# davide-coccomini/MINTIME-Multi-Identity-size-iNvariant-TIMEsformer-for-Video-Deepfake-Detection

Measured on AMD Instinct MI355X. Metric: clips/sec (8-frame, 2-identity, 224^2 crops) fwd+bwd, higher is better.
Workload: dtype f32; 1 GPU; config 3: EfficientNet-B0 + SizeInvariantTimeSformer(dim 512, depth 9, heads 8), B=32/GPU, 8 frames, 2 identities (identity-masked), 224x224 crops, random-init seeded weights (restored before every step), train-mode BN + drop-connect 0.2, step = fwd + BCE loss + bwd + SGD(lr .01, wd 1e-4); global_batch=32, frames=8, parallelism=dp1

## Files before the change

### mintime-multi-identity-size-invariant-timesformer-for-video-deepfake-detection_amd/csrc/tsf_bwd.hip

```cpp
#include "../../include/mintime_hip.h"
#include "common.hpp"
#include <stdlib.h>
#include <float.h>

using namespace mt;

#include "planes.hpp"
#include "det.hpp"
namespace {

constexpr int DH = 64;

template <int NI>
__global__ __launch_bounds__(256) void layernorm_bwd_kernel(const float* __restrict__ dy, const float* __restrict__ x,
                                                            const float* __restrict__ stats, const float* __restrict__ gamma,
                                                            float* __restrict__ dx, float* __restrict__ dgamma,
                                                            float* __restrict__ dbeta, int rows, int D, int accumulate,
                                                            float* __restrict__ dxsum, int skip_period, const float* dx_in, const DetLog det) {
  const int lane = threadIdx.x & 63;
  const int wave_global = blockIdx.x * 4 + (threadIdx.x >> 6);
  const int nwaves = gridDim.x * 4;
  const int nq = D >> 2;
  float4 dg[NI], db[NI], g[NI], ds[NI];
#pragma unroll
  for (int i = 0; i < NI; ++i) {
    dg[i] = make_float4(0.f, 0.f, 0.f, 0.f); db[i] = dg[i]; ds[i] = dg[i];
    const int q = lane + i * 64;
    g[i] = q < nq ? reinterpret_cast<const float4*>(gamma)[q] : make_float4(0.f, 0.f, 0.f, 0.f);
  }
  for (int row0 = wave_global; row0 < rows; row0 += 2 * nwaves) {
    const int row1 = row0 + nwaves;
    const bool has1 = row1 < rows;
    const int r1 = has1 ? row1 : row0;
    const float mean0 = stats[2 * (int64_t)row0], rstd0 = stats[2 * (int64_t)row0 + 1];
    const float mean1 = stats[2 * (int64_t)r1], rstd1 = stats[2 * (int64_t)r1 + 1];
    const float4* xr0 = reinterpret_cast<const float4*>(x + (int64_t)row0 * D);
    const float4* dyr0 = reinterpret_cast<const float4*>(dy + (int64_t)row0 * D);
    const float4* xr1 = reinterpret_cast<const float4*>(x + (int64_t)r1 * D);
    const float4* dyr1 = reinterpret_cast<const float4*>(dy + (int64_t)r1 * D);
    float4 xh0[NI], gy0[NI], xh1[NI], gy1[NI];
    float a1 = 0.f, a2 = 0.f, b1 = 0.f, b2 = 0.f;
    const float w1 = has1 ? 1.f : 0.f;
#pragma unroll
    for (int i = 0; i < NI; ++i) {
      const int q = lane + i * 64;
      if (q < nq) {
        const float4 xv0 = xr0[q], d0 = dyr0[q], xv1 = xr1[q], d1 = dyr1[q];
        xh0[i] = make_float4((xv0.x - mean0) * rstd0, (xv0.y - mean0) * rstd0, (xv0.z - mean0) * rstd0, (xv0.w - mean0) * rstd0);
        xh1[i] = make_float4((xv1.x - mean1) * rstd1, (xv1.y - mean1) * rstd1, (xv1.z - mean1) * rstd1, (xv1.w - mean1) * rstd1);
        gy0[i] = make_float4(d0.x * g[i].x, d0.y * g[i].y, d0.z * g[i].z, d0.w * g[i].w);
        gy1[i] = make_float4(d1.x * g[i].x, d1.y * g[i].y, d1.z * g[i].z, d1.w * g[i].w);
        a1 += gy0[i].x + gy0[i].y + gy0[i].z + gy0[i].w;
        a2 += gy0[i].x * xh0[i].x + gy0[i].y * xh0[i].y + gy0[i].z * xh0[i].z + gy0[i].w * xh0[i].w;
        b1 += gy1[i].x + gy1[i].y + gy1[i].z + gy1[i].w;
        b2 += gy1[i].x * xh1[i].x + gy1[i].y * xh1[i].y + gy1[i].z * xh1[i].z + gy1[i].w * xh1[i].w;
        dg[i].x += d0.x * xh0[i].x + w1 * d1.x * xh1[i].x; dg[i].y += d0.y * xh0[i].y + w1 * d1.y * xh1[i].y;
        dg[i].z += d0.z * xh0[i].z + w1 * d1.z * xh1[i].z; dg[i].w += d0.w * xh0[i].w + w1 * d1.w * xh1[i].w;
        db[i].x += d0.x + w1 * d1.x; db[i].y += d0.y + w1 * d1.y; db[i].z += d0.z + w1 * d1.z; db[i].w += d0.w + w1 * d1.w;
      }
    }
    a1 = wave_sum(a1) / (float)D; a2 = wave_sum(a2) / (float)D;
    b1 = wave_sum(b1) / (float)D; b2 = wave_sum(b2) / (float)D;
    float4* dxr0 = reinterpret_cast<float4*>(dx + (int64_t)row0 * D);
    float4* dxr1 = reinterpret_cast<float4*>(dx + (int64_t)r1 * D);
    const float4* pin0 = reinterpret_cast<const float4*>(dx_in + (int64_t)row0 * D);
    const float4* pin1 = reinterpret_cast<const float4*>(dx_in + (int64_t)r1 * D);
    const float c0 = (skip_period > 0 && row0 % skip_period == 0) ? 0.f : 1.f;
    const float c1 = (!has1 || (skip_period > 0 && row1 % skip_period == 0)) ? 0.f : 1.f;
#pragma unroll
    for (int i = 0; i < NI; ++i) {
      const int q = lane + i * 64;
      if (q < nq) {
        float4 o;
        o.x = rstd0 * (gy0[i].x - a1 - xh0[i].x * a2); o.y = rstd0 * (gy0[i].y - a1 - xh0[i].y * a2);
        o.z = rstd0 * (gy0[i].z - a1 - xh0[i].z * a2); o.w = rstd0 * (gy0[i].w - a1 - xh0[i].w * a2);
        if (accumulate) { const float4 p = pin0[q]; o.x += p.x; o.y += p.y; o.z += p.z; o.w += p.w; }
        dxr0[q] = o;
        ds[i].x += c0 * o.x; ds[i].y += c0 * o.y; ds[i].z += c0 * o.z; ds[i].w += c0 * o.w;
        if (has1) {
          float4 t;
          t.x = rstd1 * (gy1[i].x - b1 - xh1[i].x * b2); t.y = rstd1 * (gy1[i].y - b1 - xh1[i].y * b2);
          t.z = rstd1 * (gy1[i].z - b1 - xh1[i].z * b2); t.w = rstd1 * (gy1[i].w - b1 - xh1[i].w * b2);
          if (accumulate) { const float4 p = pin1[q]; t.x += p.x; t.y += p.y; t.z += p.z; t.w += p.w; }
          dxr1[q] = t;
          ds[i].x += c1 * t.x; ds[i].y += c1 * t.y; ds[i].z += c1 * t.z; ds[i].w += c1 * t.w;
        }
      }
    }
  }
  __shared__ float red[4][1024];
  const int wv = threadIdx.x >> 6;
#pragma unroll 1
  for (int which = 0; which < 3; ++which) {
    if (which == 2 && !dxsum) break;
#pragma unroll
    for (int i = 0; i < NI; ++i) {
      const int q = lane + i * 64;
      if (q < nq) *reinterpret_cast<float4*>(&red[wv][4 * q]) = which == 0 ? dg[i] : (which == 1 ? db[i] : ds[i]);
    }
    __syncthreads();
    float* dst = which == 0 ? dgamma : (which == 1 ? dbeta : dxsum);
    for (int c = threadIdx.x; c < D; c += 256) {
      const float v = red[0][c] + red[1][c] + red[2][c] + red[3][c];
      if (det.vals) det_put(det, which, blockIdx.x, c, v);
      else atomicAdd(dst + c, v);
    }
    __syncthreads();
  }
}

template <int NI, bool KEEP = false>
__device__ __forceinline__ void layernorm_bwd_rows_body(const float* __restrict__ dy, const float* __restrict__ x,
                                                        const float* __restrict__ stats, const float* __restrict__ gamma,
                                                        float* __restrict__ dx, const float* __restrict__ dx_in, int rows, int D,
                                                        const PlaneRef dxp) {
  const int lane = threadIdx.x & 63;
  const int nwaves = gridDim.x * 4;
  const int nq = D >> 2;
  const float inv_d = 1.0f / (float)D;
  if (dxp.p && blockIdx.x == 0)
    for (int row = rows + (threadIdx.x >> 6); row < dxp.rows_pad; row += 4)
      for (int q = lane; q < nq; q += 64) planes_store4(dxp, row, q * 4, 0.f, 0.f, 0.f, 0.f);
  for (int row = blockIdx.x * 4 + (threadIdx.x >> 6); row < rows; row += nwaves) {
    const float mean = stats[2 * (int64_t)row], rstd = stats[2 * (int64_t)row + 1];
    const float4* xr = reinterpret_cast<const float4*>(x + (int64_t)row * D);
    const float4* dyr = reinterpret_cast<const float4*>(dy + (int64_t)row * D);
    const float4* pin = reinterpret_cast<const float4*>(dx_in + (int64_t)row * D);
    float4* dxr = reinterpret_cast<float4*>(dx + (int64_t)row * D);
    if constexpr (KEEP) {
      float4 xv[NI], d[NI], g[NI], pv[NI];
      float a1 = 0.f, a2 = 0.f;
#pragma unroll
      for (int i = 0; i < NI; ++i) {
        const int q = min(lane + i * 64, nq - 1);
        xv[i] = xr[q]; d[i] = dyr[q]; g[i] = reinterpret_cast<const float4*>(gamma)[q]; pv[i] = pin[q];
      }
#pragma unroll
      for (int i = 0; i < NI; ++i) {
        const float w = lane + i * 64 < nq ? 1.f : 0.f;
        const float gx = d[i].x * g[i].x, gy_ = d[i].y * g[i].y, gz = d[i].z * g[i].z, gw = d[i].w * g[i].w;
        a1 += w * (gx + gy_ + gz + gw);
        a2 += w * rstd * (gx * (xv[i].x - mean) + gy_ * (xv[i].y - mean) + gz * (xv[i].z - mean) + gw * (xv[i].w - mean));
      }
      a1 = wave_sum(a1) * inv_d; a2 = wave_sum(a2) * inv_d;
#pragma unroll
      for (int i = 0; i < NI; ++i) {
        const int q = lane + i * 64;
        if (q < nq) {
          float4 o;
          o.x = rstd * (d[i].x * g[i].x - a1 - (xv[i].x - mean) * rstd * a2) + pv[i].x; o.y = rstd * (d[i].y * g[i].y - a1 - (xv[i].y - mean) * rstd * a2) + pv[i].y;
          o.z = rstd * (d[i].z * g[i].z - a1 - (xv[i].z - mean) * rstd * a2) + pv[i].z; o.w = rstd * (d[i].w * g[i].w - a1 - (xv[i].w - mean) * rstd * a2) + pv[i].w;
          dxr[q] = o;
          if (dxp.p) planes_store4(dxp, row, q * 4, o.x, o.y, o.z, o.w);
        }
      }
      continue;
    }
    float a1 = 0.f, a2 = 0.f;
#pragma unroll 1
    for (int i = 0; i < NI; ++i) {
      const int q = min(lane + i * 64, nq - 1);
      const float w = lane + i * 64 < nq ? 1.f : 0.f;
      const float4 xv = xr[q], d = dyr[q], g = reinterpret_cast<const float4*>(gamma)[q];
      const float gx = d.x * g.x, gy_ = d.y * g.y, gz = d.z * g.z, gw = d.w * g.w;
      a1 += w * (gx + gy_ + gz + gw);
      a2 += w * rstd * (gx * (xv.x - mean) + gy_ * (xv.y - mean) + gz * (xv.z - mean) + gw * (xv.w - mean));
    }
    a1 = wave_sum(a1) * inv_d; a2 = wave_sum(a2) * inv_d;
#pragma unroll 1
    for (int i = 0; i < NI; ++i) {
      const int q = lane + i * 64;
      if (q < nq) {
        const float4 xv = xr[q], d = dyr[q], g = reinterpret_cast<const float4*>(gamma)[q], p = pin[q];
        float4 o;
        o.x = rstd * (d.x * g.x - a1 - (xv.x - mean) * rstd * a2) + p.x; o.y = rstd * (d.y * g.y - a1 - (xv.y - mean) * rstd * a2) + p.y;
        o.z = rstd * (d.z * g.z - a1 - (xv.z - mean) * rstd * a2) + p.z; o.w = rstd * (d.w * g.w - a1 - (xv.w - mean) * rstd * a2) + p.w;
        dxr[q] = o;
        if (dxp.p) planes_store4(dxp, row, q * 4, o.x, o.y, o.z, o.w);
      }
    }
  }
}

__global__ __launch_bounds__(256) void layernorm_bwd_rows_kernel2k(
    const float* dy, const float* x, const float* stats, const float* gamma, float* dx, const float* dx_in, int rows, int D, PlaneRef dxp) {
  layernorm_bwd_rows_body<2, true>(dy, x, stats, gamma, dx, dx_in, rows, D, dxp);
}
__global__ __launch_bounds__(256) void layernorm_bwd_rows_kernel4(const float* dy, const float* x, const float* stats, const float* gamma,
                                                                   float* dx, const float* dx_in, int rows, int D, PlaneRef dxp) {
  layernorm_bwd_rows_body<4>(dy, x, stats, gamma, dx, dx_in, rows, D, dxp);
}

__global__ __launch_bounds__(256) void layernorm_bwd_rows_sums_kernel(
    const float* __restrict__ dy, const float* __restrict__ x, const float* __restrict__ stats, const float* __restrict__ gamma,
    float* __restrict__ dx, const float* __restrict__ dx_in, int rows, int D, PlaneRef dxp, float* __restrict__ partials, int skip_period) {
  constexpr int NI = 2;
  const int lane = threadIdx.x & 63, wv = threadIdx.x >> 6;
  const int nwaves = gridDim.x * 4;
  const int nq = D >> 2;
  const float inv_d = 1.0f / (float)D;
  if (dxp.p && blockIdx.x == 0)
    for (int row = rows + wv; row < dxp.rows_pad; row += 4)
      for (int q = lane; q < nq; q += 64) planes_store4(dxp, row, q * 4, 0.f, 0.f, 0.f, 0.f);
  float4 dg[NI], db[NI], ds[NI];
#pragma unroll
  for (int i = 0; i < NI; ++i) { dg[i] = make_float4(0.f, 0.f, 0.f, 0.f); db[i] = dg[i]; ds[i] = dg[i]; }
  for (int row = blockIdx.x * 4 + wv; row < rows; row += nwaves) {
    const float mean = stats[2 * (int64_t)row], rstd = stats[2 * (int64_t)row + 1];
    const float keep = (skip_period > 0 && row % skip_period == 0) ? 0.f : 1.f;
    const float4* xr = reinterpret_cast<const float4*>(x + (int64_t)row * D);
    const float4* dyr = reinterpret_cast<const float4*>(dy + (int64_t)row * D);
    const float4* pin = reinterpret_cast<const float4*>(dx_in + (int64_t)row * D);
    float4* dxr = reinterpret_cast<float4*>(dx + (int64_t)row * D);
    float4 xv[NI], d[NI], g[NI], pv[NI];
    float a1 = 0.f, a2 = 0.f;
#pragma unroll
    for (int i = 0; i < NI; ++i) {
      const int q = min(lane + i * 64, nq - 1);
      xv[i] = xr[q]; d[i] = dyr[q]; g[i] = reinterpret_cast<const float4*>(gamma)[q]; pv[i] = pin[q];
    }
#pragma unroll
    for (int i = 0; i < NI; ++i) {
      const float w = lane + i * 64 < nq ? 1.f : 0.f;
      xv[i].x = (xv[i].x - mean) * rstd; xv[i].y = (xv[i].y - mean) * rstd; xv[i].z = (xv[i].z - mean) * rstd; xv[i].w = (xv[i].w - mean) * rstd;
      const float gx = d[i].x * g[i].x, gy_ = d[i].y * g[i].y, gz = d[i].z * g[i].z, gw = d[i].w * g[i].w;
      a1 += w * (gx + gy_ + gz + gw);
      a2 += w * (gx * xv[i].x + gy_ * xv[i].y + gz * xv[i].z + gw * xv[i].w);
    }
    a1 = wave_sum(a1) * inv_d; a2 = wave_sum(a2) * inv_d;
#pragma unroll
    for (int i = 0; i < NI; ++i) {
      const int q = lane + i * 64;
      if (q < nq) {
        float4 o;
        o.x = rstd * (d[i].x * g[i].x - a1 - xv[i].x * a2) + pv[i].x; o.y = rstd * (d[i].y * g[i].y - a1 - xv[i].y * a2) + pv[i].y;
        o.z = rstd * (d[i].z * g[i].z - a1 - xv[i].z * a2) + pv[i].z; o.w = rstd * (d[i].w * g[i].w - a1 - xv[i].w * a2) + pv[i].w;
        dxr[q] = o;
        if (dxp.p) planes_store4(dxp, row, q * 4, o.x, o.y, o.z, o.w);
        dg[i].x += d[i].x * xv[i].x; dg[i].y += d[i].y * xv[i].y; dg[i].z += d[i].z * xv[i].z; dg[i].w += d[i].w * xv[i].w;
        db[i].x += d[i].x; db[i].y += d[i].y; db[i].z += d[i].z; db[i].w += d[i].w;
        ds[i].x += keep * o.x; ds[i].y += keep * o.y; ds[i].z += keep * o.z; ds[i].w += keep * o.w;
      }
    }
  }
  __shared__ float red[4][512];
  auto meet = [&](const float4 (&v)[NI], int which) {
#pragma unroll
    for (int i = 0; i < NI; ++i) {
      const int q = lane + i * 64;
      if (q < nq) *reinterpret_cast<float4*>(&red[wv][4 * q]) = v[i];
    }
    __syncthreads();
    float* dst = partials + ((int64_t)blockIdx.x * 3 + which) * D;
    for (int c = threadIdx.x; c < D; c += 256) dst[c] = red[0][c] + red[1][c] + red[2][c] + red[3][c];
    __syncthreads();
  };
  meet(dg, 0);
  meet(db, 1);
  meet(ds, 2);
}

__global__ __launch_bounds__(1024) void layernorm_cols_reduce_kernel(const float* __restrict__ partials, int blocks, int D,
                                                                     float* __restrict__ dgamma, float* __restrict__ dbeta,
                                                                     float* __restrict__ dxsum) {
  const int which = blockIdx.y;
  float* dst = which == 0 ? dgamma : (which == 1 ? dbeta : dxsum);
  if (!dst) return;
  __shared__ float red[16][64];
  const int cl = threadIdx.x & 63, ph = threadIdx.x >> 6;
  const int c = blockIdx.x * 64 + cl;
  float s0 = 0.f, s1 = 0.f, s2 = 0.f, s3 = 0.f;
  if (c < D) {
    const float* src = partials + (int64_t)which * D + c;
    const int64_t stride = (int64_t)3 * D;
    int b = ph;
    for (; b + 48 < blocks; b += 64) {
      s0 += src[(int64_t)b * stride]; s1 += src[(int64_t)(b + 16) * stride];
      s2 += src[(int64_t)(b + 32) * stride]; s3 += src[(int64_t)(b + 48) * stride];
    }
    for (; b < blocks; b += 16) s0 += src[(int64_t)b * stride];
  }
  red[ph][cl] = (s0 + s1) + (s2 + s3);
  __syncthreads();
  if (ph == 0 && c < D) {
    float t = 0.f;
#pragma unroll
    for (int q = 0; q < 16; ++q) t += red[q][cl];
    dst[c] += t;
  }
}

template <int NI>
__global__ __launch_bounds__(256) void layernorm_bwd_cols_kernel(const float* __restrict__ dy, const float* __restrict__ x,
                                                                 const float* __restrict__ stats, const float* __restrict__ dxn,
                                                                 float* __restrict__ dgamma, float* __restrict__ dbeta,
                                                                 float* __restrict__ dxsum, int skip_period, int rows, int D, const DetLog det) {
  const int lane = threadIdx.x & 63;
  const int nwaves = gridDim.x * 4;
  const int nq = D >> 2;
  float4 dg[NI], db[NI], ds[NI];
#pragma unroll
  for (int i = 0; i < NI; ++i) { dg[i] = make_float4(0.f, 0.f, 0.f, 0.f); db[i] = dg[i]; ds[i] = dg[i]; }
  for (int row = blockIdx.x * 4 + (threadIdx.x >> 6); row < rows; row += nwaves) {
    const float mean = stats[2 * (int64_t)row], rstd = stats[2 * (int64_t)row + 1];
    const float c = (skip_period > 0 && row % skip_period == 0) ? 0.f : 1.f;
#pragma unroll
    for (int i = 0; i < NI; ++i) {
      const int q = lane + i * 64;
      if (q < nq) {
        const float4 xv = reinterpret_cast<const float4*>(x + (int64_t)row * D)[q];
        const float4 d = reinterpret_cast<const float4*>(dy + (int64_t)row * D)[q];
        dg[i].x += d.x * ((xv.x - mean) * rstd); dg[i].y += d.y * ((xv.y - mean) * rstd);
        dg[i].z += d.z * ((xv.z - mean) * rstd); dg[i].w += d.w * ((xv.w - mean) * rstd);
        db[i].x += d.x; db[i].y += d.y; db[i].z += d.z; db[i].w += d.w;
        if (dxsum) {
          const float4 o = reinterpret_cast<const float4*>(dxn + (int64_t)row * D)[q];
          ds[i].x += c * o.x; ds[i].y += c * o.y; ds[i].z += c * o.z; ds[i].w += c * o.w;
        }
      }
    }
  }
  __shared__ float red[4][1024];
  const int wv = threadIdx.x >> 6;
#pragma unroll 1
  for (int which = 0; which < 3; ++which) {
    if (which == 2 && !dxsum) break;
#pragma unroll
    for (int i = 0; i < NI; ++i) {
      const int q = lane + i * 64;
      if (q < nq) *reinterpret_cast<float4*>(&red[wv][4 * q]) = which == 0 ? dg[i] : (which == 1 ? db[i] : ds[i]);
    }
    __syncthreads();
    float* dst = which == 0 ? dgamma : (which == 1 ? dbeta : dxsum);
    for (int cidx = threadIdx.x; cidx < D; cidx += 256) {
      const float v = red[0][cidx] + red[1][cidx] + red[2][cidx] + red[3][cidx];
      if (det.vals) det_put(det, which, blockIdx.x, cidx, v);
      else atomicAdd(dst + cidx, v);
    }
    __syncthreads();
  }
}

__global__ __launch_bounds__(256) void colsum_kernel(const float* __restrict__ A, int64_t lda, int gin, int gout, int off,
                                                     int M, int N, float* __restrict__ out, int rows_per_block, const DetLog det) {
  __shared__ float red[4][64];
  const int cl = threadIdx.x & 63, rl = threadIdx.x >> 6;
  const int n = blockIdx.x * 64 + cl;
  const int m0 = blockIdx.y * rows_per_block;
  const int m1 = min(M, m0 + rows_per_block);
  float s = 0.f;
  if (n < N) {
    for (int m = m0 + rl; m < m1; m += 4) {
      int64_t r = m;
      if (gin) { const int g = m / gin; r = (int64_t)g * gout + off + (m - g * gin); }
      s += A[r * lda + n];
    }
  }
  red[rl][cl] = s;
  __syncthreads();
  if (rl == 0 && n < N) {
    const float v = red[0][cl] + red[1][cl] + red[2][cl] + red[3][cl];
    if (det.vals) {
      det_put(det, blockIdx.x, blockIdx.y, cl, v);
      if (blockIdx.y == 0 && cl == 0) det_base(det, blockIdx.x, (int64_t)blockIdx.x * 64);
    } else atomicAdd(out + n, v);
  }
}

__global__ void head_bwd_kernel(const float* __restrict__ dlogits, const float* __restrict__ x, const float* __restrict__ gamma,
                                const float* __restrict__ beta, const float* __restrict__ w, float* __restrict__ dx,
                                float* __restrict__ dgamma, float* __restrict__ dbeta, float* __restrict__ dw,
                                float* __restrict__ dbias, int B, int N, int D, int C, float eps) {
  __shared__ float red[2][16];
  const int i = threadIdx.x;
  const int lane = i & 63, wv = i >> 6, nw = blockDim.x >> 6;
  auto block_sum2 = [&](float a, float b, float& oa, float& ob) {
    a = wave_sum(a); b = wave_sum(b);
    __syncthreads();
    if (lane == 0) { red[0][wv] = a; red[1][wv] = b; }
    __syncthreads();
    float sa = 0.f, sb = 0.f;
    for (int k = 0; k < nw; ++k) { sa += red[0][k]; sb += red[1][k]; }
    oa = sa; ob = sb;
  };
  float dg = 0.f, db = 0.f;
  const float gi = gamma[i], bi = beta[i];
  for (int b = 0; b < B; ++b) {
    const float xv = x[(int64_t)b * N * D + i];
    float s, dummy;
    block_sum2(xv, 0.f, s, dummy);
    const float mean = s / (float)D;
    float ss;
    block_sum2((xv - mean) * (xv - mean), 0.f, ss, dummy);
    const float rstd = rsqrtf(ss / (float)D + eps);
    const float xh = (xv - mean) * rstd;
    const float xn = xh * gi + bi;
    float dxn = 0.f;
    for (int c = 0; c < C; ++c) {
      const float dl = dlogits[b * C + c];
      dxn += dl * w[(int64_t)c * D + i];
      dw[(int64_t)c * D + i] += dl * xn;
    }
    dg += dxn * xh; db += dxn;
    const float gy = dxn * gi;
    float c1, c2;
    block_sum2(gy, gy * xh, c1, c2);
    c1 /= (float)D; c2 /= (float)D;
    dx[(int64_t)b * N * D + i] = rstd * (gy - c1 - xh * c2);
  }
  dgamma[i] += dg; dbeta[i] += db;
  if (i < C) {
    float s = 0.f;
    for (int b = 0; b < B; ++b) s += dlogits[b * C + i];
    dbias[i] += s;
  }
}

__global__ void head_bwd_clips_kernel(const float* __restrict__ dlogits, const float* __restrict__ x, const float* __restrict__ gamma,
                                      const float* __restrict__ beta, const float* __restrict__ w, float* __restrict__ dx,
                                      float* __restrict__ dgamma, float* __restrict__ dbeta, float* __restrict__ dw,
                                      float* __restrict__ dbias, int B, int N, int D, int C, float eps) {
  __shared__ float red[2][16];
  const int i = threadIdx.x, b = blockIdx.x;
  const int lane = i & 63, wv = i >> 6, nw = blockDim.x >> 6;
  auto block_sum2 = [&](float a, float c, float& oa, float& oc) {
    a = wave_sum(a); c = wave_sum(c);
    __syncthreads();
    if (lane == 0) { red[0][wv] = a; red[1][wv] = c; }
    __syncthreads();
    float sa = 0.f, sc = 0.f;
    for (int k = 0; k < nw; ++k) { sa += red[0][k]; sc += red[1][k]; }
    oa = sa; oc = sc;
  };
  const float gi = gamma[i], bi = beta[i];
  const float xv = x[(int64_t)b * N * D + i];
  float s, dummy;
  block_sum2(xv, 0.f, s, dummy);
  const float mean = s / (float)D;
  float ss;
  block_sum2((xv - mean) * (xv - mean), 0.f, ss, dummy);
  const float rstd = rsqrtf(ss / (float)D + eps);
  const float xh = (xv - mean) * rstd;
  const float xn = xh * gi + bi;
  float dxn = 0.f;
  for (int c = 0; c < C; ++c) {
    const float dl = dlogits[b * C + c];
    dxn += dl * w[(int64_t)c * D + i];
    atomicAdd(dw + (int64_t)c * D + i, dl * xn);
  }
  atomicAdd(dgamma + i, dxn * xh);
  atomicAdd(dbeta + i, dxn);
  const float gy = dxn * gi;
  float c1, c2;
  block_sum2(gy, gy * xh, c1, c2);
  c1 /= (float)D; c2 /= (float)D;
  dx[(int64_t)b * N * D + i] = rstd * (gy - c1 - xh * c2);
  if (i < C) atomicAdd(dbias + i, dlogits[b * C + i]);
}

__global__ __launch_bounds__(256) void embed_bwd_slots_kernel(const float* __restrict__ dx, float* __restrict__ dcls,
                                                              float* __restrict__ dpos, float* __restrict__ dsize,
                                                              const int64_t* __restrict__ positions, const int* __restrict__ sizes,
                                                              int B, int N, int n, int F, int D, int pos_rows, int size_rows) {
  const int b = blockIdx.x / F, f = blockIdx.x - b * F;
  int si = sizes ? sizes[b * F + f] : 0;
  si = si < 0 ? 0 : (si >= size_rows ? size_rows - 1 : si);
  const int row0 = b * N + 1 + f * n;
  for (int i = threadIdx.x; i < D; i += 256) {
    float acc = 0.f;
#pragma unroll 7
    for (int t = 0; t < n; ++t) {
      const int row = row0 + t;
      const float v = dx[(int64_t)row * D + i];
      acc += v;
      if (dpos) {
        int64_t pi = positions ? positions[row] : (int64_t)(1 + f * n + t);
        pi = pi < 0 ? 0 : (pi >= pos_rows ? pos_rows - 1 : pi);
        atomicAdd(dpos + pi * D + i, v);
      }
    }
    if (dsize) atomicAdd(dsize + (int64_t)si * D + i, acc);
    if (f == 0) {
      const int row = b * N;
      const float v = dx[(int64_t)row * D + i];
      if (dcls) atomicAdd(dcls + i, v);
      if (dpos) {
        int64_t pi = positions ? positions[row] : 0;
        pi = pi < 0 ? 0 : (pi >= pos_rows ? pos_rows - 1 : pi);
        atomicAdd(dpos + pi * D + i, v);
      }
      if (dsize) atomicAdd(dsize + i, v);
    }
  }
}

__global__ __launch_bounds__(64) void embed_bwd_det_kernel(const float* __restrict__ dx, float* __restrict__ dcls, int B, int N, int D) {
  const int col = blockIdx.x * 64 + threadIdx.x;
  if (col >= D || !dcls) return;
  float acc = 0.f;
  for (int b = 0; b < B; ++b) acc += dx[(int64_t)b * N * D + col];
  dcls[col] += acc;
}

__global__ __launch_bounds__(256) void embed_bwd_limb_scatter_kernel(const float* __restrict__ dx, const int64_t* __restrict__ positions,
                                                                    const int* __restrict__ sizes, int B, int N, int n, int F, int D,
                                                                    int rows, int kind, double* __restrict__ acc, int64_t limb) {
  const int row = blockIdx.x * 4 + (threadIdx.x >> 6);
  const int lane = threadIdx.x & 63;
  if (row >= B * N) return;
  const int b = row / N, t = row - b * N;
  int64_t idx;
  if (kind == 1) idx = positions ? positions[row] : (int64_t)t;
  else idx = (t > 0 && sizes) ? sizes[b * F + (t - 1) / n] : 0;
  idx = idx < 0 ? 0 : (idx >= rows ? rows - 1 : idx);
  const float* dr = dx + (int64_t)row * D;
  for (int i = lane; i < D; i += 64) stat_add(acc + idx * D + i, limb, dr[i]);
}

__global__ __launch_bounds__(256) void embed_bwd_limb_decode_kernel(const double* __restrict__ acc, int64_t limb, float* __restrict__ dst,
                                                                   int64_t total) {
  for (int64_t i = (int64_t)blockIdx.x * 256 + threadIdx.x; i < total; i += (int64_t)gridDim.x * 256) {
    const long long hi = *reinterpret_cast<const long long*>(acc + i), lo = *reinterpret_cast<const long long*>(acc + limb + i);
    if (hi | lo) dst[i] += (float)stat_get(acc + i, limb);
  }
}

#ifndef MT_CLS_W
#define MT_CLS_W 16
#endif
constexpr int CLS_W = MT_CLS_W;

__device__ __forceinline__ int64_t cls_fact_off(int which, int h, int H, int j, int N, int inner, int ld) {
  const int R = (N + inner - 1) / inner;
  return (int64_t)(1 + (which * H + h) * R + j / inner) * ld + (j % inner);
}

__device__ __forceinline__ float mul_unfused(float a, float b) {
#pragma clang fp contract(off)
  return a * b;
}

__global__ __launch_bounds__(CLS_W * 64) void attn_cls_bwd_kernel(const float* __restrict__ qkv, const float* __restrict__ dout,
                                                                 float* __restrict__ dqkv, const uint8_t* __restrict__ mask,
                                                                 int B, int H, int F, int n, float scale, int factored) {
  extern __shared__ __attribute__((aligned(16))) float lds[];
  const int tid = threadIdx.x, lane = tid & 63, wave = tid >> 6;
  const int sub = tid & 15, grp = tid >> 4;
  constexpr int KPP = CLS_W * 4;
  const int bh = blockIdx.x, h = bh % H, b = bh / H;
  const int N = 1 + F * n, inner = H * DH, ld = 3 * inner;
  float* pl_ = lds;
  float* ds_ = lds + N;
  float* red = ds_ + N;
  float* part = lds + ((2 * N + CLS_W + 3) & ~3);
  const float* base = qkv + (int64_t)b * N * ld + h * DH + sub * 4;
  float* dbase = dqkv + (int64_t)b * N * ld + h * DH + sub * 4;
  float4 q = *reinterpret_cast<const float4*>(base);
  q.x *= scale; q.y *= scale; q.z *= scale; q.w *= scale;
  const float4 dO = *reinterpret_cast<const float4*>(dout + (int64_t)b * N * inner + h * DH + sub * 4);
  constexpr int CLS_U = 4;
  for (int j0 = grp; j0 < N; j0 += KPP * CLS_U) {
    float4 kk[CLS_U], vv[CLS_U];
// ... 1136 lines not shown
```

Baseline: 731.8 clips/s.

## Rework layernorm backward sums kernel with LDS accumulators and scalarized addressing

```diff
diff --git a/mintime-multi-identity-size-invariant-timesformer-for-video-deepfake-detection_amd/csrc/tsf_bwd.hip b/mintime-multi-identity-size-invariant-timesformer-for-video-deepfake-detection_amd/csrc/tsf_bwd.hip
--- a/mintime-multi-identity-size-invariant-timesformer-for-video-deepfake-detection_amd/csrc/tsf_bwd.hip
+++ b/mintime-multi-identity-size-invariant-timesformer-for-video-deepfake-detection_amd/csrc/tsf_bwd.hip
@@ -191,73 +191,122 @@
   layernorm_bwd_rows_body<4>(dy, x, stats, gamma, dx, dx_in, rows, D, dxp);
 }
 
-__global__ __launch_bounds__(256) void layernorm_bwd_rows_sums_kernel(
+
+template <int M>
+__device__ __forceinline__ float swizzle_xor_add(float v) {
+  return v + __builtin_bit_cast(float, __builtin_amdgcn_ds_swizzle(__builtin_bit_cast(int, v), (M << 10) | 0x1f));
+}
+__device__ __forceinline__ float wave_sum_uniform(float v, int lane) {
+  v += __builtin_bit_cast(float, __builtin_amdgcn_ds_bpermute((lane ^ 32) << 2, __builtin_bit_cast(int, v)));
+  v = swizzle_xor_add<16>(v); v = swizzle_xor_add<8>(v); v = swizzle_xor_add<4>(v); v = swizzle_xor_add<2>(v); v = swizzle_xor_add<1>(v);
+  return __builtin_bit_cast(float, __builtin_amdgcn_readfirstlane(__builtin_bit_cast(int, v)));
+}
+
+__device__ __forceinline__ void planes_store4_at(__bf16* rowbase, int64_t pstride, uint32_t lane_elems, float v0, float v1, float v2, float v3) {
+  bf16x2_t a0, b0, c0, a1, b1, c1;
+  split2(f32x2_t{v0, v1}, a0, b0, c0);
+  split2(f32x2_t{v2, v3}, a1, b1, c1);
+  *reinterpret_cast<bf16x4_t*>(rowbase + lane_elems) = bf16x4_t{a0[0], a0[1], a1[0], a1[1]};
+  *reinterpret_cast<bf16x4_t*>(rowbase + pstride + lane_elems) = bf16x4_t{b0[0], b0[1], b1[0], b1[1]};
+  *reinterpret_cast<bf16x4_t*>(rowbase + 2 * pstride + lane_elems) = bf16x4_t{c0[0], c0[1], c1[0], c1[1]};
+}
+
+__global__ __launch_bounds__(256, 8) void layernorm_bwd_rows_sums_kernel(
     const float* __restrict__ dy, const float* __restrict__ x, const float* __restrict__ stats, const float* __restrict__ gamma,
     float* __restrict__ dx, const float* __restrict__ dx_in, int rows, int D, PlaneRef dxp, float* __restrict__ partials, int skip_period) {
   constexpr int NI = 2;
-  const int lane = threadIdx.x & 63, wv = threadIdx.x >> 6;
+  __shared__ float4 sh[128];
+  __shared__ float4 acc[3][128];
+  const int lane = threadIdx.x & 63;
+  const int wv = __builtin_amdgcn_readfirstlane(threadIdx.x >> 6);
   const int nwaves = gridDim.x * 4;
   const int nq = D >> 2;
-  const float inv_d = 1.0f / (float)D;
+  const float inv_d = __builtin_bit_cast(float, __builtin_amdgcn_readfirstlane(__builtin_bit_cast(int, 1.0f / (float)D)));
+  if ((int)threadIdx.x < nq) sh[threadIdx.x] = reinterpret_cast<const float4*>(gamma)[threadIdx.x];
+  for (int i = threadIdx.x; i < 3 * 128; i += 256) (&acc[0][0])[i] = make_float4(0.f, 0.f, 0.f, 0.f);
   if (dxp.p && blockIdx.x == 0)
     for (int row = rows + wv; row < dxp.rows_pad; row += 4)
       for (int q = lane; q < nq; q += 64) planes_store4(dxp, row, q * 4, 0.f, 0.f, 0.f, 0.f);
-  float4 dg[NI], db[NI], ds[NI];
-#pragma unroll
-  for (int i = 0; i < NI; ++i) { dg[i] = make_float4(0.f, 0.f, 0.f, 0.f); db[i] = dg[i]; ds[i] = dg[i]; }
-  for (int row = blockIdx.x * 4 + wv; row < rows; row += nwaves) {
-    const float mean = stats[2 * (int64_t)row], rstd = stats[2 * (int64_t)row + 1];
-    const float keep = (skip_period > 0 && row % skip_period == 0) ? 0.f : 1.f;
-    const float4* xr = reinterpret_cast<const float4*>(x + (int64_t)row * D);
-    const float4* dyr = reinterpret_cast<const float4*>(dy + (int64_t)row * D);
-    const float4* pin = reinterpret_cast<const float4*>(dx_in + (int64_t)row * D);
-    float4* dxr = reinterpret_cast<float4*>(dx + (int64_t)row * D);
-    float4 xv[NI], d[NI], g[NI], pv[NI];
-    float a1 = 0.f, a2 = 0.f;
-#pragma unroll
-    for (int i = 0; i < NI; ++i) {
-      const int q = min(lane + i * 64, nq - 1);
-      xv[i] = xr[q]; d[i] = dyr[q]; g[i] = reinterpret_cast<const float4*>(gamma)[q]; pv[i] = pin[q];
-    }
-#pragma unroll
-    for (int i = 0; i < NI; ++i) {
-      const float w = lane + i * 64 < nq ? 1.f : 0.f;
-      xv[i].x = (xv[i].x - mean) * rstd; xv[i].y = (xv[i].y - mean) * rstd; xv[i].z = (xv[i].z - mean) * rstd; xv[i].w = (xv[i].w - mean) * rstd;
-      const float gx = d[i].x * g[i].x, gy_ = d[i].y * g[i].y, gz = d[i].z * g[i].z, gw = d[i].w * g[i].w;
-      a1 += w * (gx + gy_ + gz + gw);
-      a2 += w * (gx * xv[i].x + gy_ * xv[i].y + gz * xv[i].z + gw * xv[i].w);
-    }
-    a1 = wave_sum(a1) * inv_d; a2 = wave_sum(a2) * inv_d;
-#pragma unroll
-    for (int i = 0; i < NI; ++i) {
-      const int q = lane + i * 64;
-      if (q < nq) {
-        float4 o;
-        o.x = rstd * (d[i].x * g[i].x - a1 - xv[i].x * a2) + pv[i].x; o.y = rstd * (d[i].y * g[i].y - a1 - xv[i].y * a2) + pv[i].y;
-        o.z = rstd * (d[i].z * g[i].z - a1 - xv[i].z * a2) + pv[i].z; o.w = rstd * (d[i].w * g[i].w - a1 - xv[i].w * a2) + pv[i].w;
-        dxr[q] = o;
-        if (dxp.p) planes_store4(dxp, row, q * 4, o.x, o.y, o.z, o.w);
-        dg[i].x += d[i].x * xv[i].x; dg[i].y += d[i].y * xv[i].y; dg[i].z += d[i].z * xv[i].z; dg[i].w += d[i].w * xv[i].w;
-        db[i].x += d[i].x; db[i].y += d[i].y; db[i].z += d[i].z; db[i].w += d[i].w;
-        ds[i].x += keep * o.x; ds[i].y += keep * o.y; ds[i].z += keep * o.z; ds[i].w += keep * o.w;
-      }
-    }
-  }
-  __shared__ float red[4][512];
-  auto meet = [&](const float4 (&v)[NI], int which) {
-#pragma unroll
-    for (int i = 0; i < NI; ++i) {
-      const int q = lane + i * 64;
-      if (q < nq) *reinterpret_cast<float4*>(&red[wv][4 * q]) = v[i];
-    }
-    __syncthreads();
-    float* dst = partials + ((int64_t)blockIdx.x * 3 + which) * D;
-    for (int c = threadIdx.x; c < D; c += 256) dst[c] = red[0][c] + red[1][c] + red[2][c] + red[3][c];
-    __syncthreads();
-  };
-  meet(dg, 0);
-  meet(db, 1);
-  meet(ds, 2);
+  __syncthreads();
+  for (int row0 = blockIdx.x * 4; row0 < rows; row0 += nwaves) {
+    const int row = row0 + wv;
+    const bool has = row < rows;
+    const bool keep = !(skip_period > 0 && row % skip_period == 0);
+    float4 xv[NI], d[NI], pv[NI];
+    if (has) {
+#pragma clang fp contract(off)
+      const float mean = stats[2 * (int64_t)row], rstd = stats[2 * (int64_t)row + 1];
+      const uint64_t rb = (uint64_t)row * (uint64_t)D * 4u;
+      const uint64_t roff = (uint64_t)(uint32_t)__builtin_amdgcn_readfirstlane((int)(uint32_t)rb) |
+                            ((uint64_t)(uint32_t)__builtin_amdgcn_readfirstlane((int)(uint32_t)(rb >> 32)) << 32);
+      const char* xr = reinterpret_cast<const char*>(x) + roff;
+      const char* dyr = reinterpret_cast<const char*>(dy) + roff;
+      const char* pin = reinterpret_cast<const char*>(dx_in) + roff;
+      char* dxr = reinterpret_cast<char*>(dx) + roff;
+      float a1 = 0.f, a2 = 0.f;
+#pragma unroll
+      for (int i = 0; i < NI; ++i) {
+        const uint32_t qb = (uint32_t)min(lane + i * 64, nq - 1) << 4;
+        xv[i] = *reinterpret_cast<const float4*>(xr + qb); d[i] = *reinterpret_cast<const float4*>(dyr + qb);
+        pv[i] = *reinterpret_cast<const float4*>(pin + qb);
+      }
+#pragma unroll
+      for (int i = 0; i < NI; ++i) {
+        const float w = lane + i * 64 < nq ? 1.f : 0.f;
+        const float4 g = sh[min(lane + i * 64, nq - 1)];
+        xv[i].x = (xv[i].x - mean) * rstd; xv[i].y = (xv[i].y - mean) * rstd; xv[i].z = (xv[i].z - mean) * rstd; xv[i].w = (xv[i].w - mean) * rstd;
+        const float gx = d[i].x * g.x, gy_ = d[i].y * g.y, gz = d[i].z * g.z, gw = d[i].w * g.w;
+        a1 += w * (gx + gy_ + gz + gw);
+        a2 += w * (gx * xv[i].x + gy_ * xv[i].y + gz * xv[i].z + gw * xv[i].w);
+      }
+#pragma unroll
+      for (int i = 0; i < NI; ++i) asm volatile("" : "+v"(pv[i].x), "+v"(pv[i].y), "+v"(pv[i].z), "+v"(pv[i].w) : : "memory");
+      a1 = wave_sum_uniform(a1, lane) * inv_d; a2 = wave_sum_uniform(a2, lane) * inv_d;
+      __bf16* prow = dxp.p + (((int64_t)(row >> 5) * dxp.cb16) * 512 + (row & 31) * 16);
+#pragma unroll
+      for (int i = 0; i < NI; ++i) {
+        const int q = lane + i * 64;
+        if (q < nq) {
+          const float4 g = sh[q];
+          pv[i].x = __builtin_fmaf(rstd, __builtin_fmaf(-a2, xv[i].x, d[i].x * g.x - a1), pv[i].x);
+          pv[i].y = __builtin_fmaf(rstd, __builtin_fmaf(-a2, xv[i].y, d[i].y * g.y - a1), pv[i].y);
+          pv[i].z = __builtin_fmaf(rstd, __builtin_fmaf(-a2, xv[i].z, d[i].z * g.z - a1), pv[i].z);
+          pv[i].w = __builtin_fmaf(rstd, __builtin_fmaf(-a2, xv[i].w, d[i].w * g.w - a1), pv[i].w);
+          *reinterpret_cast<float4*>(dxr + ((uint32_t)q << 4)) = pv[i];
+          if (dxp.p) planes_store4_at(prow, dxp.pstride, (uint32_t)(((q >> 2) << 9) | ((q & 3) << 2)), pv[i].x, pv[i].y, pv[i].z, pv[i].w);
+        }
+      }
+    }
+#pragma unroll
+    for (int p = 0; p < 4; ++p) {
+      const int sec = (wv + p) & 3;
+      if (has && (lane >> 5) == (sec & 1)) {
+        auto add_row = [&](const float4& dd, const float4& xh, const float4& o, int q) {
+          if (q < nq) {
+            float4 t = acc[0][q];
+            t.x = __builtin_fmaf(dd.x, xh.x, t.x); t.y = __builtin_fmaf(dd.y, xh.y, t.y);
+            t.z = __builtin_fmaf(dd.z, xh.z, t.z); t.w = __builtin_fmaf(dd.w, xh.w, t.w);
+            acc[0][q] = t;
+            t = acc[1][q];
+            t.x += dd.x; t.y += dd.y; t.z += dd.z; t.w += dd.w;
+            acc[1][q] = t;
+            if (keep) {
+              t = acc[2][q];
+              t.x += o.x; t.y += o.y; t.z += o.z; t.w += o.w;
+              acc[2][q] = t;
+            }
+          }
+        };
+        if (sec >> 1) add_row(d[1], xv[1], pv[1], lane + 64);
+        else add_row(d[0], xv[0], pv[0], lane);
+      }
+      __syncthreads();
+    }
+  }
+  for (int c = threadIdx.x; c < D; c += 256)
+#pragma unroll
+    for (int which = 0; which < 3; ++which)
+      partials[((int64_t)blockIdx.x * 3 + which) * D + c] = reinterpret_cast<const float*>(&acc[which][0])[c];
 }
 
 __global__ __launch_bounds__(1024) void layernorm_cols_reduce_kernel(const float* __restrict__ partials, int blocks, int D,
```

Result: no change. 732.3 clips/s (median of 2 runs) (+0.1%).
